# InterDigitalInc/VersatileFilmGrain

Hardware: AMD Instinct MI355X
Metric: Mpixels/s (Y+UV) + achieved HBM GB/s vs roofline, 4320p 10-bit 4:2:0 (higher is better)
Workload: dtype u16

## Files before the change

versatilefilmgrain_amd/csrc/vfgs_host.cpp:

```cpp
#include <hip/hip_runtime.h>

#include <sys/mman.h>
#include <unistd.h>

#include <algorithm>
#include <chrono>
#if defined(__SSE2__)
#include <emmintrin.h>
#endif
#include <cstdarg>
#include <cstdio>
#include <cstdlib>
#include <cstring>
#include <mutex>
#include <string>
#include <thread>
#include <vector>

#include "../../include/vfgs_hip.h"
#include "../../include/vfgs_hip_fw.h"
#include "vfgs_fw_layout.h"
#include "vfgs_layout.h"

namespace vfgs {
// ... 1211 lines not shown
	if (stride < nblk * 16 || cstride < nblk * 16 / s.csubx)
		return fail(6, "stride %u/%u too small: whole 16-sample blocks are written (need >= %u/%u)", stride, cstride, nblk * 16, nblk * 16 / s.csubx);
	if (((uintptr_t)dY | (uintptr_t)dU | (uintptr_t)dV) & 15)
		return fail(7, "plane pointers must be 16-byte aligned");
	if ((stride * sz) % 16 || (cstride * sz) % 16)
		return fail(8, "row pitch must be a multiple of 16 bytes");
	if (s.scale_shift + s.bs < 8 || s.scale_shift + s.bs > 13)
		return fail(9, "scale_shift out of range (vfgs_hw.c:170)");
	return 0;
}

void load_seed(State& s, uint32_t seed)
{
	s.lfsr.reseed(seed << 1);
	s.seed_epoch++;
	s.rnd = s.rnd_up = s.line_rnd = s.line_rnd_up = 0;
}

struct DstGeom {
	bool out8 = false;
	unsigned stride = 0, cstride = 0;
	uint64_t ypitch = 0, cpitch = 0;
};

int run_device(const void* sY, const void* sU, const void* sV, void* dY, void* dU, void* dV, unsigned width,
               unsigned frame_y, unsigned frame_h, unsigned part_y, unsigned part_h, unsigned stride, unsigned cstride,
               unsigned nframes, uint64_t ypitch, uint64_t cpitch, hipStream_t stream, DstGeom dg = DstGeom(),
               const vfgs::FrameTable* list = nullptr,
               const uint32_t* seeds = nullptr)
{
	State& s = S();
	if (list && nframes > (unsigned)vfgs::kListFrames) return fail(19, "internal: a listed launch holds at most %d frames", vfgs::kListFrames);
	if (int e = ensure_init(-1)) return e;
	if (int e = check_geometry(s, sY, sU, sV, width, stride, cstride)) return e;
	if (!dg.out8)
	{
		if (int e = check_geometry(s, dY, dU, dV, width, stride, cstride)) return e;
	}
	else
	{
		const unsigned nb = (width + 15) / 16;
		if (s.bs == 0) return fail(16, "8-bit output needs a 10- or 12-bit path (vfgs_set_depth(10) or (12))");
		if (dg.stride < nb * 16 || dg.cstride < nb * 16 / s.csubx) return fail(6, "destination stride too small");
		if ((((uintptr_t)dY | (uintptr_t)dU | (uintptr_t)dV) & 15) || dg.stride % 16 || dg.cstride % 16 || (dg.ypitch | dg.cpitch) % 16)
			return fail(8, "destination planes, pitches and frame pitches must be multiples of 16 bytes");
	}
	if (seeds && (frame_y != 0 || !list)) return fail(19, "internal: seeds belong to lists of frames that begin at line 0");
	if (part_h == 0 && seeds && nframes) load_seed(s, seeds[nframes - 1]);
	if (part_h == 0 || nframes == 0) return 0;
	if (int e = check_luts(s)) return e;

	const unsigned nblk = (width + 15) / 16;
	const unsigned sz = s.bs ? 2 : 1;
	const uint64_t crows = (uint64_t)(part_y + part_h - 1) / s.csuby - part_y / s.csuby + 1;
	const uint64_t yext = (uint64_t)part_h * stride * sz, cext = crows * cstride * sz;
	if (yext >= 0x80000000ull || cext >= 0x80000000ull)
		return fail(15, "a plane stripe of %llu bytes exceeds the 2 GiB buffer window", (unsigned long long)yext);
	KernelArgs a{};
	a.src[0] = (const uint8_t*)sY; a.src[1] = (const uint8_t*)sU; a.src[2] = (const uint8_t*)sV;
	a.dst[0] = (uint8_t*)dY; a.dst[1] = (uint8_t*)dU; a.dst[2] = (uint8_t*)dV;
	a.y0 = (int)part_y;
	a.nblk = (int)nblk;
	const int nbr_stripe = (int)(((part_y + part_h - 1) >> 4) - (part_y >> 4) + 1);
	a.nbrows = nbr_stripe;
	a.nframes = (int)nframes;
	a.listed = list ? 1 : 0;
	a.lo2[0] = (uint32_t)(s.ymin << s.bs) * 0x10001u; a.hi2[0] = (uint32_t)(s.ymax << s.bs) * 0x10001u;
	a.lo2[1] = (uint32_t)(s.cmin << s.bs) * 0x10001u; a.hi2[1] = (uint32_t)(s.cmax << s.bs) * 0x10001u;
	a.pk_shift = s.scale_shift;
	const unsigned nparts = (nblk + vfgs::kTileBlocks - 1) / vfgs::kTileBlocks;
	int rw_shrink = 0;
	bool form_one_y = false, form_one_c = false;
	digest_pluts(s);
	const bool wide = nparts > 1;
	if (image_is_current(s, wide)) { form_one_y = s.img_one_y; form_one_c = s.img_one_c; }
	else if (s.plut_bad_c < 0) image_form(s, wide, &form_one_y, &form_one_c);
	const bool mix = mix_active();
	if (mix && s.bs == 4)
		return fail(38, "a chroma mix is active and the depth is 12: the kernels of the mix exist at 8 and 10 bit");
	if (mix && !(form_one_y && form_one_c))
		return fail(38, "a chroma mix is active and the programmed model needs a general-form pattern bank (%s rows): not supported", wide ? "wide" : "ordinary");
	if (mix && &s != &g_states[0])
		return fail(38, "a chroma mix is active: not supported on the devices of vfgs_hip_init_devices");
	for (int pass = 0; pass < 3; pass++)
	{
		long waves = 0;
		for (int pt = 0; pt < 2; pt++)
		{
			vfgs::PlaneDesc& d = a.pd[pt];
			const unsigned subx = pt ? s.csubx : 1, suby = pt ? s.csuby : 1;
			const unsigned bw = 16 / subx, rpb = 16 / suby;
			d.pitch = (pt ? cstride : stride) * sz;
			d.dpitch = dg.out8 ? (pt ? dg.cstride : dg.stride) : d.pitch;
			d.fpitch = pt ? cpitch : ypitch;
			d.dfpitch = dg.out8 ? (pt ? dg.cpitch : dg.ypitch) : d.fpitch;
			d.rowbytes = nblk * bw * sz;
			d.drowbytes = dg.out8 ? nblk * bw : d.rowbytes;
			d.nrows = pt ? (int)((part_y + part_h + suby - 1) / suby) - (int)((part_y + suby - 1) / suby) : (int)part_h;
			auto lg = [](int v) { int l = 0; while ((1 << l) < v) l++; return l; };
			const int units = (int)((d.rowbytes + 15) / 16);
			d.rw_segs = (units + 1 + vfgs::kMaxUnits - 1) / vfgs::kMaxUnits;
			int rpw = 1;
			const size_t wg_bytes = (pt == 0 && s.bs == 0 && !form_one_y) ? VFGS_RW_WG_BYTES / 2 : VFGS_RW_WG_BYTES;
			while (vfgs::kWavesPerWG * rpw * 2 <= (int)rpb && (size_t)vfgs::kWavesPerWG * rpw * d.rowbytes < wg_bytes) rpw *= 2;
			for (int i = 0; i < rw_shrink && rpw > 1; i++) rpw /= 2;
			if (nparts > 1) rpw = 1;
			d.rw_rpw = rpw;
			d.rw_splits = std::max<int>(1, (int)rpb / (vfgs::kWavesPerWG * rpw));
			d.rw_lsplits = lg(d.rw_splits);
			d.wgs = d.nrows > 0 ? nbr_stripe * d.rw_splits : 0;
			waves += (long)(pt ? 2 : 1) * d.wgs * vfgs::kWavesPerWG * nframes;
		}
		const long slots = (long)s.cu_count * 16;
		if (pass < 2 && waves * 100 < VFGS_RW_MIN_FILL_PCT * slots && (a.pd[0].rw_rpw > 1 || a.pd[1].rw_rpw > 1)) { rw_shrink++; continue; }
		break;
	}

	uint64_t first_cur = 0, first_up = 0, second_cur = 0, lo = ~0ull, hi = 0;
	if (seeds)
	{
		const uint64_t b = part_y >> 4;
		first_cur = b * nblk;
		first_up = b ? (b - 1) * nblk : 0;
	}
	auto seeded_done = [&] {
		load_seed(s, seeds[nframes - 1]);
		advance_seeds(s, 0, frame_h, nblk, 0);
	};
	for (unsigned f = 0; f < nframes && f < 2 && !seeds; f++)
	{
		StripePlan p = advance_seeds(s, frame_y, frame_h, nblk, part_y);
		if (f == 0) { first_cur = p.cur0; first_up = p.up0; }
		if (f == 1) second_cur = p.cur0;
		lo = std::min(lo, std::min(p.cur0, p.up0));
		hi = std::max(hi, p.cur0 + (uint64_t)nbr_stripe * nblk);
		hi = std::max(hi, p.up0 + nblk);
	}
	if (nframes > 2 && !seeds)
	{
		if (frame_y != 0) return fail(10, "internal: a batch of stripes that do not begin at line 0");
		const uint64_t step = second_cur - first_cur, more = (uint64_t)(nframes - 2) * step;
		s.rnd += more; s.rnd_up += more; s.line_rnd += more; s.line_rnd_up += more;
		hi = std::max(hi, second_cur + more + (uint64_t)nbr_stripe * nblk);
	}
	if (int e = upload_tables(s, stream, wide)) return e;
	HIP_TRY(s.tables_ring.use(stream));
	a.tables = (const uint8_t*)s.tables_ring.current();
	const uint64_t frame_step = nframes > 1 ? second_cur - first_cur : 0;
	const uint64_t seg_bits = 32 + (uint64_t)nblk + (uint64_t)nbr_stripe * nblk + 64;
	const unsigned seg_words = (unsigned)((seg_bits + 31) / 32) + 1;
	static const bool jump_on = [] { const char* e = getenv("VFGS_HIP_STRIPE_JUMP"); return !(e && e[0] == '0'); }();
	const bool stripes = !seeds && jump_on && nframes >= 2 && first_cur >= (uint64_t)nblk + 32 && first_up + nblk + 32 >= first_cur &&
	                     (uint64_t)seg_words * 32 * 4 <= frame_step * 3;
	s.stripe_stream_last = stripes;
	s.seeded_stream_last = seeds != nullptr;
	if (seeds)
	{
		const uint64_t seg0 = first_up;
		SeededStream::Image img{};
		HIP_TRY(s.seeded.upload(seeds, nframes, seg0, seg_words, stream, &img));
		a.stream = img.dev;
		a.stream_bytes = img.words * 4;
		a.cur_bit0 = (uint32_t)(first_cur - seg0);
		a.up_bit0 = 0;
		a.frame_bit_step = seg_words * 32;
	}
	else if (stripes)
	{
		const uint64_t seg0 = first_cur - nblk - 32;
		StripeStream::Image img{};
		HIP_TRY(s.stripes.ensure(s.lfsr, seg0, frame_step, nframes, seg_words, stream, &img));
		a.stream = img.dev;
		a.stream_bytes = img.words * 4;
		a.cur_bit0 = (uint32_t)(first_cur - seg0);
		a.up_bit0 = (uint32_t)(std::max(first_up, seg0) - seg0);
		a.frame_bit_step = seg_words * 32;
	}
	else
	{
		if (int e = upload_stream(s, lo, hi, stream)) return e;
		HIP_TRY(s.lfsr.use(stream));
		a.stream = s.lfsr.dev();
		a.stream_bytes = (uint32_t)(s.lfsr.dev_words() * 4);
		a.cur_bit0 = (uint32_t)(first_cur - s.lfsr.base_bit());
		a.up_bit0 = (uint32_t)(first_up - s.lfsr.base_bit());
		a.frame_bit_step = (uint32_t)frame_step;
	}

	const long per_frame = (long)a.pd[0].wgs + 2L * a.pd[1].wgs;
	if (per_frame > 0x3fffffffL || nframes > 65535) return fail(14, "launch too large");
	if (per_frame == 0) { if (seeds) seeded_done(); return 0; }
	bool persist = false;
	long grid = per_frame;
	if (VFGS_PERSIST_MIN_TASKS > 0 && s.bs != 0 && !wide && !s.img_one_y && a.pd[0].wgs > 0 &&
	    (size_t)vfgs::kWavesPerWG * a.pd[0].rw_rpw * a.pd[0].rowbytes <= ((size_t)VFGS_PERSIST_MAX_WG_KB << 10))
	{
		const long tasks = (long)a.pd[0].wgs * nframes, slots = (long)s.cu_count * 4;
		const long k = (tasks + slots - 1) / slots;
		if (k >= VFGS_PERSIST_MIN_TASKS)
		{
			const long P = (tasks + k - 1) / k;
			persist = true;
			a.persist_wgs = (int)P;
			a.persist_step_f = (int)(P / a.pd[0].wgs);
			a.persist_step_r = (int)(P % a.pd[0].wgs);
			grid = P + 2L * a.pd[1].wgs * nframes;
			if (grid > 0x7fffffffL) return fail(14, "launch too large");
		}
	}
#ifdef VFGS_NO_FRONTS
	a.lfronts = 0;
#else
	const bool in_region = g_states[0].ov.active && (stream == g_states[0].ov.s[0] || stream == g_states[0].ov.s[1]);
	a.lfronts = (!persist && nframes >= 2 && !in_region && 2 * (yext + 2 * cext) >= (64u << 20)) ? 1 : 0;
#endif
	if (mix)
	{
		if (!(s.img_one_y && s.img_one_c) || persist) return fail(19, "internal: the table image is not the form the chroma mix was admitted for");
		a.mix_kernel = 1;
		a.mix_lw = (int)width;
		for (int c = 0; c < 2; c++)
		{
			a.mix[c][0] = g_mix[c][0]; a.mix[c][1] = g_mix[c][1];
			a.mix[c][2] = g_mix[c][2] * (1 << s.bs);
			a.mix[c][3] = g_mix[c][3];
		}
		const uint64_t dext = dg.out8 ? (uint64_t)part_h * dg.stride : yext, dfp = dg.out8 ? dg.ypitch : ypitch;
		auto meet = [](uintptr_t p, uint64_t pn, uintptr_t q, uint64_t qn) { return p < q + qn && q < p + pn; };
		bool shared = false;
		if (!list)
			shared = meet((uintptr_t)sY, (uint64_t)(nframes - 1) * ypitch + yext, (uintptr_t)dY, (uint64_t)(nframes - 1) * dfp + dext);
		else
			for (unsigned i = 0; i < nframes && !shared; i++)
				for (unsigned j = 0; j < nframes && !shared; j++)
					shared = meet((uintptr_t)list->src[0][i], yext, (uintptr_t)list->dst[0][j], dext);
		if (shared)
		{
			a.mix_planes = 1;
			HIP_TRY(vfgs::launch_grain(a, list, 8 + s.bs, s.csubx, s.csuby, dg.out8, true, true, wide, false, (int)grid, stream));
			a.mix_planes = 2;
		}
	}
	HIP_TRY(vfgs::launch_grain(a, list, 8 + s.bs, s.csubx, s.csuby, dg.out8, s.img_one_y, s.img_one_c, wide, persist, (int)grid, stream));
	if (seeds) seeded_done();
	if (stripes && s.stripes.prepare_next(s.lfsr) != hipSuccess) (void)hipGetLastError();
	if (&s == &g_states[0])
	{
		vfgs_hip_launch_info& li = g_last_launch;
		const unsigned long long n = li.launches + 1;
		li = vfgs_hip_launch_info{};
		li.launches = n;
		li.depth = 8 + s.bs; li.csubx = s.csubx; li.csuby = s.csuby;
		li.out8 = dg.out8; li.one_y = s.img_one_y; li.one_c = s.img_one_c;
		li.in_place = (sY == dY && sU == dU && sV == dV);
		li.listed = a.listed;
		li.internal = g_internal_launch ? 1 : 0;
		li.nframes = (int)nframes;
		li.workgroups_per_frame = (int)per_frame;
		li.frames_per_front = 1 << a.lfronts;
		for (int pt = 0; pt < 2; pt++)
		{
			li.rows_per_wave[pt] = a.pd[pt].rw_rpw;
			li.positions_per_row[pt] = a.pd[pt].rw_segs;
		}
		li.parts_per_row = (int)nparts;
		li.persistent_luma_workgroups = persist ? a.persist_wgs : 0;
		li.waves_per_workgroup = vfgs::kWavesPerWG;
		const vfgs::ImageLayout L = vfgs::layout_of(s.csubx, s.csuby, s.img_one_y, s.img_one_c, s.bs == 0);
		li.lds_bytes_per_workgroup = vfgs::lds_allocation(s.bs != 0, s.img_one_y, s.img_one_c, wide, L.lds_bytes + vfgs::kParamBytes);
		vfgs::describe_launch(li.kernel, sizeof li.kernel, 8 + s.bs, s.csubx, s.csuby, dg.out8, s.img_one_y, s.img_one_c, wide, persist);
		if (mix)
		{
			li.lds_bytes_per_workgroup = vfgs::mix_lds_allocation(L.lds_bytes + vfgs::kParamBytes);
			snprintf(li.kernel, sizeof li.kernel, "grain_mix_kernel<%d,%d,%d,%s,%s>", 8 + s.bs, s.csubx, s.csuby, dg.out8 ? "true" : "false", wide ? "true" : "false");
			if (a.mix_planes) li.launches++;
		}
		g_last_launch_valid = true;
	}
	return 0;
}

int run_host(void* Y, void* U, void* V, unsigned y, unsigned width, unsigned height, unsigned stride, unsigned cstride, unsigned py, unsigned ph)
{
	State& s = S();
	if (int e = ensure_init(-1)) return e;
	if (height == 0) return 0;
	const unsigned sz = s.bs ? 2 : 1;
	const unsigned nblk = (width + 15) / 16;
	if (ph == 0)
	{
		if (int e = check_luts(s)) return e;
		advance_seeds(s, y, height, nblk, y);
		return 0;
	}
	const unsigned crow0 = py / s.csuby;
	const unsigned crows = (py + ph - 1) / s.csuby - crow0 + 1;
	const unsigned rows[3] = {ph, crows, crows};
	const unsigned rowlen[3] = {nblk * 16 * sz, nblk * 16 / s.csubx * sz, nblk * 16 / s.csubx * sz};
	const unsigned dpitch[3] = {(rowlen[0] + 255) & ~255u, (rowlen[1] + 255) & ~255u, (rowlen[2] + 255) & ~255u};
	const size_t spitch[3] = {std::max<size_t>((size_t)stride * sz, rowlen[0]), std::max<size_t>((size_t)cstride * sz, rowlen[1]),
	                          std::max<size_t>((size_t)cstride * sz, rowlen[2])};
	uint8_t* host[3] = {(uint8_t*)Y + (size_t)(py - y) * spitch[0], (uint8_t*)U + (size_t)(crow0 - y / s.csuby) * spitch[1],
	                    (uint8_t*)V + (size_t)(crow0 - y / s.csuby) * spitch[2]};
	size_t total = 0;
	for (int i = 0; i < 3; i++) total += (size_t)dpitch[i] * rows[i];
	const bool via_bounce = total <= (1u << 20);
	for (int i = 0; i < 3; i++)
	{
		const size_t need = (size_t)dpitch[i] * rows[i] + 256;
		if (s.stage_cap[i] < need)
		{
			if (s.stage[i]) HIP_TRY(hipFree(s.stage[i]));
			s.stage[i] = nullptr; s.stage_cap[i] = 0;
			HIP_TRY(hipMalloc(&s.stage[i], need));
			s.stage_cap[i] = need;
		}
		if (via_bounce)
		{
			if (s.bounce_cap[i] < need)
			{
				if (s.bounce[i]) HIP_TRY(hipHostFree(s.bounce[i]));
				s.bounce[i] = nullptr; s.bounce_cap[i] = 0;
				HIP_TRY(hipHostMalloc((void**)&s.bounce[i], std::max<size_t>(need, 64u << 10), hipHostMallocDefault));
				s.bounce_cap[i] = std::max<size_t>(need, 64u << 10);
			}
			for (unsigned r = 0; r < rows[i]; r++)
				memcpy(s.bounce[i] + (size_t)r * dpitch[i], host[i] + (size_t)r * spitch[i], rowlen[i]);
			HIP_TRY(hipMemcpyAsync(s.stage[i], s.bounce[i], (size_t)dpitch[i] * rows[i], hipMemcpyHostToDevice, s.own_stream));
		}
		else
			HIP_TRY(hipMemcpy2DAsync(s.stage[i], dpitch[i], host[i], spitch[i], rowlen[i], rows[i], hipMemcpyHostToDevice, s.own_stream));
	}
	{
		InternalLaunch mark;
		if (int e = run_device(s.stage[0], s.stage[1], s.stage[2], s.stage[0], s.stage[1], s.stage[2], width, y, height, py, ph,
		                       dpitch[0] / sz, dpitch[1] / sz, 1, 0, 0, s.own_stream))
			return e;
	}
	for (int i = 0; i < 3; i++)
	{
		if (via_bounce) HIP_TRY(hipMemcpyAsync(s.bounce[i], s.stage[i], (size_t)dpitch[i] * rows[i], hipMemcpyDeviceToHost, s.own_stream));
		else HIP_TRY(hipMemcpy2DAsync(host[i], spitch[i], s.stage[i], dpitch[i], rowlen[i], rows[i], hipMemcpyDeviceToHost, s.own_stream));
	}
	HIP_TRY(hipStreamSynchronize(s.own_stream));
	if (via_bounce)
		for (int i = 0; i < 3; i++)
			for (unsigned r = 0; r < rows[i]; r++)
				memcpy(host[i] + (size_t)r * spitch[i], s.bounce[i] + (size_t)r * dpitch[i], rowlen[i]);
	return 0;
}

int run_host(void* Y, void* U, void* V, unsigned y, unsigned width, unsigned height, unsigned stride, unsigned cstride)
{
// ... 1319 lines not shown
```

versatilefilmgrain_amd/csrc/vfgs_kernel.hip:

```cpp
#include <hip/hip_runtime.h>
#include <stdint.h>
#include <stdio.h>

#include <type_traits>

#include "vfgs_layout.h"

namespace vfgs {

typedef uint32_t u32x4 __attribute__((ext_vector_type(4)));
typedef uint32_t u32x2 __attribute__((ext_vector_type(2)));
typedef uint32_t u32x3 __attribute__((ext_vector_type(3)));
typedef short s16x2 __attribute__((ext_vector_type(2)));
typedef unsigned short u16x2 __attribute__((ext_vector_type(2)));


__device__ __forceinline__ int pick_slot(uint32_t hi, uint32_t lo, uint32_t lut_entry)
{
	return (int)__builtin_amdgcn_perm(hi, lo, lut_entry) >> 24;
}

__device__ __forceinline__ int mad_i24(int x, uint32_t y, int c)
{
	int r;
// ... 870 lines not shown
#endif
template <int DEPTH, bool ONEY, bool ONEC, bool WIDE>
constexpr int rw_waves_per_simd()
{
#ifdef VFGS_ONE10_WAVES
	if (DEPTH > 8 && ONEY && ONEC && !WIDE) return VFGS_ONE10_WAVES;
#endif
	return (DEPTH == 8 && ONEY && ONEC && !WIDE && VFGS_WG_PER_CU == 4) ? (kPk16 ? VFGS_PK_WAVES : 5) : (kWavesPerWG * VFGS_WG_PER_CU + 3) / 4;
}

template <int DEPTH, int CSUBX, int CSUBY, bool OUT8, bool ONEY, bool ONEC, bool WIDE, bool PERSIST>
__global__ __launch_bounds__(kWavesPerWG * 64, (rw_waves_per_simd<DEPTH, ONEY, ONEC, WIDE>())) void grain_rw_kernel(const KernelArgs a, const FrameTable ft)
{
	constexpr ImageLayout L = image_layout(CSUBX, CSUBY, ONEY, ONEC, DEPTH == 8);
	__shared__ __attribute__((aligned(16))) uint8_t lds[lds_allocation(DEPTH > 8, ONEY, ONEC, WIDE, L.lds_bytes + kParamBytes)];

	const int lane = threadIdx.x & 63;
	const int wave = __builtin_amdgcn_readfirstlane(threadIdx.x >> 6);
	int f, r;
	if constexpr (PERSIST)
	{
		static_assert(!ONEY && !WIDE, "persistence exists for the general-form luma image");
		if ((int)blockIdx.x < a.persist_wgs)
		{
			f = (int)blockIdx.x / a.pd[0].wgs;
			r = (int)blockIdx.x - f * a.pd[0].wgs;
			run_plane_rw<DEPTH, 16, 1, 1, L.y_rs, L.y_bytes, ONEY, L.y_neg, 0, OUT8, WIDE, true>(a, ft, a.pd[0], lds, 0, f, r, L.y_off, L.y_bank, 0, lane, wave);
			return;
		}
		const int x = (int)blockIdx.x - a.persist_wgs, per = 2 * a.pd[1].wgs;
		f = x / per;
		r = a.pd[0].wgs + (x - f * per);
	}
	else
	{
		f = (int)(blockIdx.y << a.lfronts) + (int)(blockIdx.x & ((1u << a.lfronts) - 1));
		r = (int)(blockIdx.x >> a.lfronts);
	}
	if (f >= a.nframes) return;
	if (r < a.pd[0].wgs)
		run_plane_rw<DEPTH, 16, 1, 1, L.y_rs, L.y_bytes, ONEY, L.y_neg, 0, OUT8, WIDE, false>(a, ft, a.pd[0], lds, 0, f, r, L.y_off, L.y_bank, 0, lane, wave);
	else
	{
		r -= a.pd[0].wgs;
		const int comp = 1 + (r >= a.pd[1].wgs);
		if (comp == 2) r -= a.pd[1].wgs;
		if (!WIDE && CSUBX == 2 && a.pd[1].rw_segs == 2 && ring_depth<DEPTH, ONEC>() >= 2)
			run_plane_rw<DEPTH, 16 / CSUBX, CSUBX, CSUBY, L.c_rs, L.c_bytes, ONEC, L.c_neg, WIDE ? 0 : 2, OUT8, WIDE, false>(a, ft, a.pd[1], lds, comp, f, r, L.c_off[comp - 1], L.c_bank, L.c_lut[comp - 1], lane, wave);
		else if (!WIDE && CSUBX == 2 && a.pd[1].rw_segs == 1)
			run_plane_rw<DEPTH, 16 / CSUBX, CSUBX, CSUBY, L.c_rs, L.c_bytes, ONEC, L.c_neg, WIDE ? 0 : 1, OUT8, WIDE, false>(a, ft, a.pd[1], lds, comp, f, r, L.c_off[comp - 1], L.c_bank, L.c_lut[comp - 1], lane, wave);
		else
			run_plane_rw<DEPTH, 16 / CSUBX, CSUBX, CSUBY, L.c_rs, L.c_bytes, ONEC, L.c_neg, 0, OUT8, WIDE, false>(a, ft, a.pd[1], lds, comp, f, r, L.c_off[comp - 1], L.c_bank, L.c_lut[comp - 1], lane, wave);
	}
}

template <int DEPTH, int CSUBX, int CSUBY, bool OUT8, bool WIDE>
__global__ __launch_bounds__(kWavesPerWG * 64, kMixWgPerCU) void grain_mix_kernel(const KernelArgs a, const FrameTable ft)
{
	constexpr ImageLayout L = image_layout(CSUBX, CSUBY, true, true, DEPTH == 8);
	__shared__ __attribute__((aligned(16))) uint8_t lds[mix_lds_allocation(L.lds_bytes + kParamBytes)];

	const int lane = threadIdx.x & 63;
	const int wave = __builtin_amdgcn_readfirstlane(threadIdx.x >> 6);
	const int f = (int)(blockIdx.y << a.lfronts) + (int)(blockIdx.x & ((1u << a.lfronts) - 1));
	int r = (int)(blockIdx.x >> a.lfronts);
	if (f >= a.nframes) return;
	if (r < a.pd[0].wgs)
	{
		if (a.mix_planes & 1) return;
		run_plane_rw<DEPTH, 16, 1, 1, L.y_rs, L.y_bytes, true, L.y_neg, 0, OUT8, WIDE, false>(a, ft, a.pd[0], lds, 0, f, r, L.y_off, L.y_bank, 0, lane, wave);
	}
	else
	{
		if (a.mix_planes & 2) return;
		r -= a.pd[0].wgs;
		const int n = a.pd[1].wgs, full = n & ~7;
		int comp;
		if (r < 2 * full) { comp = 1 + ((r >> 3) & 1); r = ((r >> 4) << 3) | (r & 7); }
		else { r -= 2 * full; comp = 1 + (r >= n - full); r = full + (comp == 2 ? r - (n - full) : r); }
		run_plane_rw<DEPTH, 16 / CSUBX, CSUBX, CSUBY, L.c_rs, L.c_bytes, true, L.c_neg, 0, OUT8, WIDE, false, true>(a, ft, a.pd[1], lds, comp, f, r, L.c_off[comp - 1], L.c_bank, L.c_lut[comp - 1], lane, wave);
	}
}


template <int DEPTH, int CSUBX, int CSUBY, bool OUT8>
static hipError_t launch_mix(const KernelArgs& a, const FrameTable& ft, bool wide, int grid, hipStream_t stream)
{
	const dim3 g((unsigned)grid << a.lfronts, ((unsigned)a.nframes + (1u << a.lfronts) - 1) >> a.lfronts);
	if (wide)
	{
		if constexpr (CSUBX == CSUBY) hipLaunchKernelGGL((grain_mix_kernel<DEPTH, CSUBX, CSUBY, OUT8, true>), g, dim3(kWavesPerWG * 64), 0, stream, a, ft);
		else return hipErrorInvalidValue;
	}
	else
		hipLaunchKernelGGL((grain_mix_kernel<DEPTH, CSUBX, CSUBY, OUT8, false>), g, dim3(kWavesPerWG * 64), 0, stream, a, ft);
	return hipGetLastError();
}

template <int DEPTH, int CSUBX, int CSUBY, bool OUT8, bool ONEY, bool ONEC, bool WIDE, bool PERSIST>
static hipError_t launch_t(const KernelArgs& a, const FrameTable& ft, int grid, hipStream_t stream)
{
	const dim3 g = PERSIST ? dim3((unsigned)grid) : dim3((unsigned)grid << a.lfronts, ((unsigned)a.nframes + (1u << a.lfronts) - 1) >> a.lfronts);
	hipLaunchKernelGGL((grain_rw_kernel<DEPTH, CSUBX, CSUBY, OUT8, ONEY, ONEC, WIDE, PERSIST>), g, dim3(kWavesPerWG * 64), 0, stream, a, ft);
	return hipGetLastError();
}

template <int DEPTH, int CSUBX, int CSUBY, bool OUT8>
static hipError_t launch_form(const KernelArgs& a, const FrameTable& ft, bool oney, bool onec, bool wide, bool persist, int grid, hipStream_t stream)
{
	if (wide)
	{
		if (persist) return hipErrorInvalidValue;
		if constexpr (CSUBX == CSUBY)
		{
			if (oney && onec) return launch_t<DEPTH, CSUBX, CSUBY, OUT8, true, true, true, false>(a, ft, grid, stream);
			if (!oney && onec) return launch_t<DEPTH, CSUBX, CSUBY, OUT8, false, true, true, false>(a, ft, grid, stream);
		}
		return (oney || onec) ? hipErrorInvalidValue : launch_t<DEPTH, CSUBX, CSUBY, OUT8, false, false, true, false>(a, ft, grid, stream);
	}
	if constexpr (DEPTH > 8)
	{
		if (persist)
		{
			if (oney) return hipErrorInvalidValue;
			return onec ? launch_t<DEPTH, CSUBX, CSUBY, OUT8, false, true, false, true>(a, ft, grid, stream)
			            : launch_t<DEPTH, CSUBX, CSUBY, OUT8, false, false, false, true>(a, ft, grid, stream);
		}
	}
	else if (persist) return hipErrorInvalidValue;
	if (oney && onec) return launch_t<DEPTH, CSUBX, CSUBY, OUT8, true, true, false, false>(a, ft, grid, stream);
	if (oney) return launch_t<DEPTH, CSUBX, CSUBY, OUT8, true, false, false, false>(a, ft, grid, stream);
	if (onec) return launch_t<DEPTH, CSUBX, CSUBY, OUT8, false, true, false, false>(a, ft, grid, stream);
	return launch_t<DEPTH, CSUBX, CSUBY, OUT8, false, false, false, false>(a, ft, grid, stream);
}

template <int D>
static hipError_t launch_depth(const KernelArgs& a, const FrameTable& ft, int csubx, int csuby, bool out8, bool oney, bool onec, bool wide, bool persist, int grid, hipStream_t stream)
{
	if (a.mix_kernel)
	{
		if (!oney || !onec || persist) return hipErrorInvalidValue;
#define VFGS_CASE(X, Y)                                                                                  \
	if (csubx == X && csuby == Y)                                                                        \
	{                                                                                                    \
		if constexpr (D == 10) { if (out8) return launch_mix<D, X, Y, true>(a, ft, wide, grid, stream); } \
		if constexpr (D != 12) return launch_mix<D, X, Y, false>(a, ft, wide, grid, stream);              \
	}
		VFGS_CASE(2, 2) VFGS_CASE(2, 1) VFGS_CASE(1, 1) VFGS_CASE(1, 2)
#undef VFGS_CASE
		return hipErrorInvalidValue;
	}
#define VFGS_CASE(X, Y)                                                                                                     \
	if (csubx == X && csuby == Y)                                                                                           \
	{                                                                                                                       \
		if constexpr (D > 8) { if (out8) return launch_form<D, X, Y, true>(a, ft, oney, onec, wide, persist, grid, stream); }   \
		return launch_form<D, X, Y, false>(a, ft, oney, onec, wide, persist, grid, stream);                                     \
	}
	VFGS_CASE(2, 2) VFGS_CASE(2, 1) VFGS_CASE(1, 1) VFGS_CASE(1, 2)
#undef VFGS_CASE
	return hipErrorInvalidValue;
}

#if !defined(VFGS_KERNEL_DEPTH) || VFGS_KERNEL_DEPTH == 8
hipError_t launch_grain_d8(const KernelArgs& a, const FrameTable& ft, int csubx, int csuby, bool out8, bool oney, bool onec, bool wide, bool persist, int grid, hipStream_t stream)
{
	return launch_depth<8>(a, ft, csubx, csuby, out8, oney, onec, wide, persist, grid, stream);
}
#else
hipError_t launch_grain_d8(const KernelArgs& a, const FrameTable& ft, int csubx, int csuby, bool out8, bool oney, bool onec, bool wide, bool persist, int grid, hipStream_t stream);
#endif

#if !defined(VFGS_KERNEL_DEPTH) || VFGS_KERNEL_DEPTH == 12
hipError_t launch_grain_d12(const KernelArgs& a, const FrameTable& ft, int csubx, int csuby, bool out8, bool oney, bool onec, bool wide, bool persist, int grid, hipStream_t stream)
{
	return launch_depth<12>(a, ft, csubx, csuby, out8, oney, onec, wide, persist, grid, stream);
}
#else
hipError_t launch_grain_d12(const KernelArgs& a, const FrameTable& ft, int csubx, int csuby, bool out8, bool oney, bool onec, bool wide, bool persist, int grid, hipStream_t stream);
#endif

#if !defined(VFGS_KERNEL_DEPTH) || VFGS_KERNEL_DEPTH == 10
hipError_t launch_grain(const KernelArgs& a, const FrameTable* list, int depth, int csubx, int csuby, bool out8, bool oney, bool onec, bool wide, bool persist, int grid, hipStream_t stream)
{
	if ((out8 && depth != 10 && depth != 12) || wide != (a.nblk > kTileBlocks)) return hipErrorInvalidValue;
	if (a.mix_kernel ? (a.mix_lw < 1 || a.mix_lw > a.nblk * kBlock) : a.mix_planes != 0) return hipErrorInvalidValue;
	if ((a.listed != 0) != (list != nullptr) || (list && a.nframes > kListFrames)) return hipErrorInvalidValue;
	static const FrameTable no_list{};
	const FrameTable& ft = list ? *list : no_list;
	if (depth == 10) return launch_depth<10>(a, ft, csubx, csuby, out8, oney, onec, wide, persist, grid, stream);
	if (depth == 8) return launch_grain_d8(a, ft, csubx, csuby, out8, oney, onec, wide, persist, grid, stream);
	if (depth == 12) return launch_grain_d12(a, ft, csubx, csuby, out8, oney, onec, wide, persist, grid, stream);
	return hipErrorInvalidValue;
}

void describe_launch(char* out, size_t n, int depth, int csubx, int csuby, bool out8, bool oney, bool onec, bool wide, bool persist)
{
	auto b = [](bool v) { return v ? "true" : "false"; };
	snprintf(out, n, "grain_rw_kernel<%d,%d,%d,%s,%s,%s,%s,%s>", depth, csubx, csuby, b(out8), b(oney), b(onec), b(wide), b(persist));
}

ImageLayout layout_of(int csubx, int csuby, bool oney, bool onec, bool depth8) { return image_layout(csubx, csuby, oney, onec, depth8); }
#endif

}
```

versatilefilmgrain_amd/csrc/vfgs_layout.h:

```cpp
#pragma once
#include <stdint.h>

namespace vfgs {

constexpr int kSlots = 8;
constexpr int kMaxUnits = 64;
constexpr int kBlock = 16;

#ifndef VFGS_WAVES
#define VFGS_WAVES 4
#endif
#ifndef VFGS_WG_PER_CU
#define VFGS_WG_PER_CU 4
#endif
#ifndef VFGS_SCHED_FENCE
#define VFGS_SCHED_FENCE 1
#endif
#ifndef VFGS_LDAUX_ALIGNED
#define VFGS_LDAUX_ALIGNED 2
#endif
#ifndef VFGS_STAUX_ALIGNED
#define VFGS_STAUX_ALIGNED 2
#endif
#ifndef VFGS_RING
#define VFGS_RING 4
#endif
#ifndef VFGS_RING_ONE10
#define VFGS_RING_ONE10 4
#endif
#ifndef VFGS_RING_PK
#define VFGS_RING_PK 2
#endif
#ifndef VFGS_RING_NARROW10
#define VFGS_RING_NARROW10 2
#endif
#ifndef VFGS_ONE10_WG_PER_CU
#define VFGS_ONE10_WG_PER_CU 4
#endif
#ifndef VFGS_ONE8_WG_PER_CU
#define VFGS_ONE8_WG_PER_CU 0
#endif
#ifndef VFGS_RW_CONSEC
#define VFGS_RW_CONSEC 0
#endif

#if !defined(VFGS_DEV_BUILD)
#if VFGS_WAVES != 4 || VFGS_WG_PER_CU != 4 || VFGS_RING != 4 || VFGS_RING_ONE10 != 4 || VFGS_RING_PK != 2 || VFGS_RING_NARROW10 != 2 || VFGS_ONE10_WG_PER_CU != 4 || VFGS_ONE8_WG_PER_CU != 0 || VFGS_SCHED_FENCE != 1 || VFGS_LDAUX_ALIGNED != 2 || VFGS_STAUX_ALIGNED != 2 || VFGS_RW_CONSEC != 0 || \
    defined(VFGS_NO_FRONTS) || defined(VFGS_NO_LOOKAHEAD) || defined(VFGS_NO_ONE_PATTERN) || defined(VFGS_NO_PK16) || defined(VFGS_PK_NO_READ2) || defined(VFGS_PK_WAVES) || defined(VFGS_ONE10_WAVES) ||  defined(VFGS_RW_WG_BYTES) || defined(VFGS_RW_MIN_FILL_PCT) || defined(VFGS_PERSIST_MIN_TASKS) || defined(VFGS_PERSIST_MAX_WG_KB)
#error "libvfgs_hip: a tuning knob differs from the shipped configuration; developer variants must define VFGS_DEV_BUILD"
#endif
#endif

constexpr int kWavesPerWG = VFGS_WAVES;
#ifdef VFGS_NO_PK16
constexpr bool kPk16 = false;
#else
constexpr bool kPk16 = true;
#endif

constexpr int kTileBlocks = 512;
constexpr int kParamEntries = kTileBlocks + 4;
constexpr int kParamTableBytes = (kParamEntries * 4 + 15) & ~15;
constexpr int kParamBytes = 2 * kParamTableBytes;

constexpr int kLdsPerCU = 163840;
constexpr int lds_allocation(const bool depth10, const bool one_y, const bool one_c, const bool wide, const int need)
{
	const int cap = (depth10 && one_y) ? VFGS_ONE10_WG_PER_CU : ((!depth10 && one_y && one_c && !wide) ? VFGS_ONE8_WG_PER_CU : 0);
	if (cap <= 0) return need;
	const int target = (kLdsPerCU / cap) & ~2047;
	const int next = (kLdsPerCU / (cap + 1)) & ~2047;
	return need > next ? need : (target < 65536 ? target : 65536);
}

constexpr int kMixWgPerCU = 4;
constexpr int mix_lds_allocation(const int need)
{
	const int target = (kLdsPerCU / kMixWgPerCU) & ~2047;
	return need > target ? need : target;
}

struct ImageLayout {
	int lut_bytes;
	int y_rs, c_rs;
	int y_bank, c_bank;
	int y_neg, c_neg;
	int y_bytes, c_bytes;
	int y_off, c_off[2];
	int c_lut[2];
	int bytes;
	int lds_bytes;
	int cw, ch;
};

constexpr ImageLayout image_layout(int csubx, int csuby, bool one_y, bool one_c, bool depth8)
{
	ImageLayout L{};
	L.lut_bytes = 2 * 256 * 4;
	L.cw = 64 / csubx;
	L.ch = 64 / csuby;
	depth8 = depth8 && kPk16;
	const int ob = depth8 ? 2 : 1;
	L.y_rs = one_y ? 64 * ob + 16 : 64 * kSlots + 16;
	L.c_rs = one_c ? L.cw * ob + 16 : L.cw * kSlots + 16;
	L.y_bank = one_y ? (depth8 ? 256 : L.lut_bytes / 2) : L.lut_bytes;
	L.c_bank = one_c ? (depth8 ? 256 : L.lut_bytes / 2) : L.lut_bytes;
	L.y_neg = one_y ? 64 * L.y_rs : 0;
	L.c_neg = one_c ? L.ch * L.c_rs : 0;
	L.y_bytes = L.y_bank + 64 * L.y_rs + L.y_neg;
	L.c_bytes = L.c_bank + L.ch * L.c_rs + L.c_neg;
	L.y_off = 0;
	L.c_off[0] = L.y_bytes;
	L.c_off[1] = L.y_bytes + L.c_bytes;
	L.c_lut[0] = 0;
	L.c_lut[1] = 0;
	L.bytes = L.y_bytes + 2 * L.c_bytes;
	L.lds_bytes = L.y_bytes > L.c_bytes ? L.y_bytes : L.c_bytes;
	return L;
}

struct PlaneDesc {
	uint32_t pitch, dpitch;
	uint64_t fpitch, dfpitch;
	uint32_t rowbytes, drowbytes;
	int nrows;
	int wgs;
	int rw_segs;
	int rw_rpw, rw_splits, rw_lsplits;
};

constexpr int kListFrames = 32;
struct FrameTable {
	const uint8_t* src[3][kListFrames];
	uint8_t* dst[3][kListFrames];
};

struct KernelArgs {
	const uint8_t* src[3];
	uint8_t* dst[3];
	PlaneDesc pd[2];
	const uint32_t* stream;
	uint32_t stream_bytes;
	const uint8_t* tables;
	uint32_t cur_bit0;
	uint32_t up_bit0;
	uint32_t frame_bit_step;
	int y0;
	int nblk;
	int nbrows;
	int nframes;
	int listed;
	int lfronts;
	int persist_wgs;
	int persist_step_f, persist_step_r;
	int pk_shift;
	uint32_t lo2[2], hi2[2];
	int mix_kernel;
	int mix_planes;
	int mix_lw;
	int mix[2][4];
};

}
```

Measured before the change: 963,500.

## Add per-row luma workgroups for 10-bit 4:2:0 wide frames

Adds a new grain_row_kernel in which each luma workgroup handles exactly one pixel row. It loads into LDS only the bank rows that row needs (16 rows instead of the full 64-row pattern bank), which shrinks LDS per workgroup so more workgroups fit per CU (five by default). Chroma still goes through the existing row-wave path inside the same kernel. The host selects this form for 10-bit 4:2:0, general-form luma with 385 to 512 blocks per row, which covers 4320p, and disables the persistent schedule for it. In exchange, each workgroup repeats per-row setup work (bank load and block-parameter decode) 16 times per block row, and the kernel adds new DPP lane-shift code.

```diff
diff --git a/versatilefilmgrain_amd/csrc/vfgs_host.cpp b/versatilefilmgrain_amd/csrc/vfgs_host.cpp
--- a/versatilefilmgrain_amd/csrc/vfgs_host.cpp
+++ b/versatilefilmgrain_amd/csrc/vfgs_host.cpp
@@ -1317,6 +1317,7 @@
 		return fail(38, "a chroma mix is active and the programmed model needs a general-form pattern bank (%s rows): not supported", wide ? "wide" : "ordinary");
 	if (mix && &s != &g_states[0])
 		return fail(38, "a chroma mix is active: not supported on the devices of vfgs_hip_init_devices");
+	const bool rowwg = !mix && !wide && vfgs::row_form(8 + s.bs, s.csubx, s.csuby, form_one_y, dg.out8, (int)nblk);
 	for (int pass = 0; pass < 3; pass++)
 	{
 		long waves = 0;
@@ -1342,6 +1343,7 @@
 			if (nparts > 1) rpw = 1;
 			d.rw_rpw = rpw;
 			d.rw_splits = std::max<int>(1, (int)rpb / (vfgs::kWavesPerWG * rpw));
+			if (pt == 0 && rowwg) { d.rw_rpw = 1; d.rw_splits = (int)rpb; }
 			d.rw_lsplits = lg(d.rw_splits);
 			d.wgs = d.nrows > 0 ? nbr_stripe * d.rw_splits : 0;
 			waves += (long)(pt ? 2 : 1) * d.wgs * vfgs::kWavesPerWG * nframes;
@@ -1427,7 +1429,8 @@
 	if (per_frame == 0) { if (seeds) seeded_done(); return 0; }
 	bool persist = false;
 	long grid = per_frame;
-	if (VFGS_PERSIST_MIN_TASKS > 0 && s.bs != 0 && !wide && !s.img_one_y && a.pd[0].wgs > 0 &&
+	if (rowwg && s.img_one_y) return fail(19, "internal: the table image is not the form the row workgroups were chosen for");
+	if (VFGS_PERSIST_MIN_TASKS > 0 && s.bs != 0 && !wide && !rowwg && !s.img_one_y && a.pd[0].wgs > 0 &&
 	    (size_t)vfgs::kWavesPerWG * a.pd[0].rw_rpw * a.pd[0].rowbytes <= ((size_t)VFGS_PERSIST_MAX_WG_KB << 10))
 	{
 		const long tasks = (long)a.pd[0].wgs * nframes, slots = (long)s.cu_count * 4;
@@ -1476,6 +1479,7 @@
 			a.mix_planes = 2;
 		}
 	}
+	a.row_wgs = rowwg ? 1 : 0;
 	HIP_TRY(vfgs::launch_grain(a, list, 8 + s.bs, s.csubx, s.csuby, dg.out8, s.img_one_y, s.img_one_c, wide, persist, (int)grid, stream));
 	if (seeds) seeded_done();
 	if (stripes && s.stripes.prepare_next(s.lfsr) != hipSuccess) (void)hipGetLastError();
@@ -1504,6 +1508,11 @@
 		const vfgs::ImageLayout L = vfgs::layout_of(s.csubx, s.csuby, s.img_one_y, s.img_one_c, s.bs == 0);
 		li.lds_bytes_per_workgroup = vfgs::lds_allocation(s.bs != 0, s.img_one_y, s.img_one_c, wide, L.lds_bytes + vfgs::kParamBytes);
 		vfgs::describe_launch(li.kernel, sizeof li.kernel, 8 + s.bs, s.csubx, s.csuby, dg.out8, s.img_one_y, s.img_one_c, wide, persist);
+		if (rowwg)
+		{
+			li.lds_bytes_per_workgroup = vfgs::row_lds_allocation(vfgs::row_lds_need(s.img_one_c));
+			snprintf(li.kernel, sizeof li.kernel, "grain_row_kernel<%d,%s>", 8 + s.bs, s.img_one_c ? "true" : "false");
+		}
 		if (mix)
 		{
 			li.lds_bytes_per_workgroup = vfgs::mix_lds_allocation(L.lds_bytes + vfgs::kParamBytes);
diff --git a/versatilefilmgrain_amd/csrc/vfgs_kernel.hip b/versatilefilmgrain_amd/csrc/vfgs_kernel.hip
--- a/versatilefilmgrain_amd/csrc/vfgs_kernel.hip
+++ b/versatilefilmgrain_amd/csrc/vfgs_kernel.hip
@@ -976,6 +976,188 @@
 	}
 }
 
+template <int DEPTH, int RS>
+__device__ __forceinline__ void run_luma_row(const KernelArgs& a, const FrameTable& ft, uint8_t* lds, const int f, const int r,
+                                             const uint32_t img_off, const uint32_t src_bank, const uint32_t img_bytes, const int lane, const int wave)
+{
+	static_assert(DEPTH == 10, "row workgroups exist at 10 bit");
+	using M = LaneMap<8, 16>;
+	static_assert(M::PAIR && M::SHIFT * 2 / 4 == 4, "the lane shift is a whole unit");
+	constexpr int SB = kSlots;
+	constexpr int LDA = VFGS_LDAUX_ALIGNED, STA = VFGS_STAUX_ALIGNED;
+	constexpr int NU = 4;
+	constexpr int BPS = 32, SSTEP = 64;
+	constexpr uint32_t UB = kMaxUnits * 16;
+	constexpr uint32_t BANK = 2 * 256 * 4;
+	constexpr int RU = RS / 16;
+	constexpr int IMG_UNITS = (int)BANK / 16 + kRowBankRows * RU;
+	constexpr uint32_t PT_CUR = IMG_UNITS * 16, PT_UP = PT_CUR + kParamTableBytes;
+	static_assert(RS % 16 == 0, "bank rows in whole 16-byte units");
+	const PlaneDesc& pd = a.pd[0];
+	auto uni = [](int v) { return __builtin_amdgcn_readfirstlane(v); };
+
+	const int kbr = uni(r >> 4), j = uni(r & 15);
+	const int Rabs = (a.y0 >> 4) + kbr;
+	const int row = Rabs * 16 + j;
+	if (kbr >= a.nbrows || row < a.y0 || row >= a.y0 + pd.nrows) return;
+	const bool ov = Rabs > 0 && j <= 1;
+	const int last = a.nblk - 1;
+	const uint32_t cur_bit = a.cur_bit0 + (uint32_t)f * a.frame_bit_step + (uint32_t)(kbr * a.nblk);
+	const uint32_t up_bit = (kbr > 0) ? cur_bit - (uint32_t)a.nblk : a.up_bit0 + (uint32_t)f * a.frame_bit_step;
+
+	constexpr int STEP = kWavesPerWG * 64;
+	constexpr int NIT = (IMG_UNITS + STEP - 1) / STEP;
+	u32x4 tmp[NIT];
+	const __amdgpu_buffer_rsrc_t irs = make_rsrc(a.tables + img_off, img_bytes);
+#pragma unroll
+	for (int it = 0; it < NIT; it++)
+	{
+		const uint32_t i = min((uint32_t)threadIdx.x + it * STEP, (uint32_t)IMG_UNITS - 1);
+		const uint32_t bi = i - BANK / 16, c = bi / RU, col = bi - c * RU;
+		const uint32_t so = i < BANK / 16 ? i * 16 : src_bank + ((4 * c + (uint32_t)(j & 3)) * RU + col) * 16;
+		tmp[it] = __builtin_amdgcn_raw_buffer_load_b128(irs, so, 0, 0);
+	}
+	constexpr int NPE = (kParamEntries + STEP - 1) / STEP;
+	const __amdgpu_buffer_rsrc_t strs = make_rsrc((const uint8_t*)a.stream, a.stream_bytes);
+	const __amdgpu_buffer_rsrc_t strs_up = make_rsrc((const uint8_t*)a.stream, ov ? a.stream_bytes : 0);
+	u32x2 wc[NPE], wu[NPE];
+#pragma unroll
+	for (int i = 0; i < NPE; i++)
+	{
+		const int e = (int)threadIdx.x + i * STEP;
+		const uint32_t blk = (uint32_t)min(max(e - 1, 0), last);
+		const bool need = e < a.nblk + 4 && e < kParamEntries;
+		wc[i] = __builtin_amdgcn_raw_buffer_load_b64(strs, need ? ((cur_bit + blk) >> 5) * 4 : kOOB, 0, 0);
+		wu[i] = __builtin_amdgcn_raw_buffer_load_b64(strs_up, need ? ((up_bit + blk) >> 5) * 4 : kOOB, 0, 0);
+	}
+	const int tsegs = pd.rw_segs;
+	const int p0 = NU * wave;
+	const uint8_t* sbase = a.listed ? ft.src[0][f] : a.src[0] + (uint64_t)f * pd.fpitch;
+	uint8_t* dbase = a.listed ? ft.dst[0][f] : a.dst[0] + (uint64_t)f * pd.dfpitch;
+	const uint32_t ro = (uint32_t)((row - a.y0) * (int)pd.pitch);
+	const uint32_t lane16 = (uint32_t)lane * 16;
+	const uint32_t po = (uint32_t)p0 * UB;
+	const uint32_t mine = po < pd.rowbytes ? min(pd.rowbytes - po, NU * UB) : 0u;
+	const __amdgpu_buffer_rsrc_t srow = make_rsrc(sbase + ro, pd.rowbytes), drow = make_rsrc(dbase + ro, pd.rowbytes);
+	const __amdgpu_buffer_rsrc_t src = make_rsrc(sbase + ro + po, mine), dst = make_rsrc(dbase + ro + po, mine);
+	uint32_t carry[4];
+	load_seg<LDA>(srow, (lane == 0 && wave > 0) ? po - 16 : kOOB, 0, carry);
+	uint32_t w[NU][4];
+#pragma unroll
+	for (int u = 0; u < NU; u++) load_seg<LDA>(src, lane16 + u * UB, 0, w[u]);
+#pragma unroll
+	for (int it = 0; it < NIT; it++)
+		*(u32x4*)(lds + min((uint32_t)threadIdx.x + it * STEP, (uint32_t)IMG_UNITS - 1) * 16) = tmp[it];
+
+#pragma unroll
+	for (int i = 0; i < NPE; i++)
+	{
+		if (i > 0 && i * STEP >= a.nblk + 4) break;
+		const int e = (int)threadIdx.x + i * STEP;
+		const uint32_t blk = (uint32_t)min(max(e - 1, 0), last);
+		bool neg;
+		const uint32_t vc = __builtin_amdgcn_alignbit(wc[i].y, wc[i].x, (cur_bit + blk) & 31);
+		const uint32_t pc = block_param<1, 4, RS, SB>(vc, BANK, 0, 14, 31, &neg) | (neg ? 0x80000000u : 0u);
+		const uint32_t vu = __builtin_amdgcn_alignbit(wu[i].y, wu[i].x, (up_bit + blk) & 31);
+		const uint32_t pu = block_param<1, 4, RS, SB>(vu, BANK, 0, 14, 31, &neg) | (neg ? 0x80000000u : 0u);
+		if (e < kParamEntries)
+		{
+			*(uint32_t*)(lds + PT_CUR + e * 4) = pc;
+			if (ov) *(uint32_t*)(lds + PT_UP + e * 4) = pu;
+		}
+	}
+	__syncthreads();
+
+	const uint32_t lo2 = a.lo2[0], hi2 = a.hi2[0];
+	const bool first = lane & 1;
+	const uint32_t pairoff = first ? 0u : 8u * SB;
+	const uint8_t* pe = lds + ((uint32_t)(lane + 1) >> 1) * 4 + (uint32_t)(p0 * BPS * 4);
+	const int cl = lane - 1 - (lane & 1) + p0 * SSTEP;
+	const uint32_t rowoff = (uint32_t)(j >> 2) * RS, uprowoff = (uint32_t)(4 + (j >> 2)) * RS;
+	const int wc_ = j == 0 ? 12 : 24, wu_ = j == 0 ? 24 : 12;
+	auto lane_up = [](uint32_t old, uint32_t v) { return (uint32_t)__builtin_amdgcn_update_dpp((int)old, (int)v, 0x138, 0xf, 0xf, false); };
+	auto lane_down = [](uint32_t old, uint32_t v) { return (uint32_t)__builtin_amdgcn_update_dpp((int)old, (int)v, 0x130, 0xf, 0xf, false); };
+	auto rot_up = [](uint32_t v) { return (uint32_t)__builtin_amdgcn_mov_dpp((int)v, 0x13c, 0xf, 0xf, false); };
+	auto rot_down = [](uint32_t v) { return (uint32_t)__builtin_amdgcn_mov_dpp((int)v, 0x134, 0xf, 0xf, false); };
+
+	uint32_t outp[4], tp[4] = {0, 0, 0, 0};
+	auto step = [&](auto overlap, auto uc) {
+		constexpr bool OV = decltype(overlap)::value;
+		constexpr int u = decltype(uc)::value;
+		uint32_t t[4];
+		if constexpr (u < NU)
+		{
+#pragma unroll
+			for (int d = 0; d < 4; d++) t[d] = lane_up(carry[d], w[u][d]);
+#pragma unroll
+			for (int d = 0; d < 4; d++) carry[d] = rot_up(w[u][d]);
+		}
+		else
+		{
+#pragma unroll
+			for (int d = 0; d < 4; d++) t[d] = lane_up(carry[d], 0u);
+		}
+		if (p0 + u < tsegs)
+		{
+			const int jl = cl + u * SSTEP;
+			const bool edge_on[1] = {jl >= 0 && jl + 1 < 2 * a.nblk};
+			RunParam<1> rp, up;
+			const uint8_t* pu = u < NU ? pe + u * BPS * 4 : lds + min((uint32_t)(lane + 1) >> 1, (uint32_t)(kParamEntries - 1 - kTileBlocks)) * 4 + kTileBlocks * 4;
+			rp.pa[0] = *(const uint32_t*)(pu + PT_CUR) + pairoff;
+			up.pa[0] = OV ? *(const uint32_t*)(pu + PT_UP) + pairoff : 0u;
+			grain_unit<DEPTH, 16, OV, false, false, 0>(lds, t, rp, up, 0u, rowoff, uprowoff, OV ? wc_ : 0, OV ? wu_ : 0, edge_on, first, lo2, hi2, 0, t);
+		}
+#pragma unroll
+		for (int d = 0; d < 4; d++) outp[d] = lane_down(rot_down(t[d]), tp[d]);
+		if constexpr (u == 0) store_unit<4, STA>(drow, (lane == 63 && wave > 0) ? po - 16 : kOOB, outp);
+		else store_unit<4, STA>(dst, lane16 + (u - 1) * UB, outp);
+#pragma unroll
+		for (int d = 0; d < 4; d++) tp[d] = t[d];
+#if VFGS_SCHED_FENCE
+		__builtin_amdgcn_sched_barrier(0);
+#endif
+	};
+	auto walk = [&](auto overlap) {
+		step(overlap, std::integral_constant<int, 0>());
+		step(overlap, std::integral_constant<int, 1>());
+		step(overlap, std::integral_constant<int, 2>());
+		step(overlap, std::integral_constant<int, 3>());
+		if (p0 + NU < tsegs && wave == kWavesPerWG - 1)
+			step(overlap, std::integral_constant<int, 4>());
+		else
+		{
+#pragma unroll
+			for (int d = 0; d < 4; d++) outp[d] = lane_down(0u, tp[d]);
+			store_unit<4, STA>(dst, lane == 63 ? kOOB : lane16 + (NU - 1) * UB, outp);
+		}
+	};
+	if (ov) walk(std::true_type());
+	else walk(std::false_type());
+}
+
+template <int DEPTH, bool ONEC>
+__global__ __launch_bounds__(kWavesPerWG * 64, VFGS_ROW_WG_PER_CU) void grain_row_kernel(const KernelArgs a, const FrameTable ft)
+{
+	static_assert(kWavesPerWG == 4, "wave w walks positions 4w..4w+3 of a row of at most 17");
+	constexpr ImageLayout L = image_layout(2, 2, false, ONEC, false);
+	__shared__ __attribute__((aligned(16))) uint8_t lds[row_lds_allocation(row_lds_need(ONEC))];
+
+	const int lane = threadIdx.x & 63;
+	const int wave = __builtin_amdgcn_readfirstlane(threadIdx.x >> 6);
+	const int f = (int)(blockIdx.y << a.lfronts) + (int)(blockIdx.x & ((1u << a.lfronts) - 1));
+	int r = (int)(blockIdx.x >> a.lfronts);
+	if (f >= a.nframes) return;
+	if (r < a.pd[0].wgs)
+		run_luma_row<DEPTH, L.y_rs>(a, ft, lds, f, r, L.y_off, L.y_bank, L.y_bytes, lane, wave);
+	else
+	{
+		r -= a.pd[0].wgs;
+		const int comp = 1 + (r >= a.pd[1].wgs);
+		if (comp == 2) r -= a.pd[1].wgs;
+		run_plane_rw<DEPTH, 8, 2, 2, L.c_rs, L.c_bytes, ONEC, L.c_neg, 0, false, false, false>(a, ft, a.pd[1], lds, comp, f, r, L.c_off[comp - 1], L.c_bank, L.c_lut[comp - 1], lane, wave);
+	}
+}
+
 
 template <int DEPTH, int CSUBX, int CSUBY, bool OUT8>
 static hipError_t launch_mix(const KernelArgs& a, const FrameTable& ft, bool wide, int grid, hipStream_t stream)
@@ -996,6 +1178,15 @@
 {
 	const dim3 g = PERSIST ? dim3((unsigned)grid) : dim3((unsigned)grid << a.lfronts, ((unsigned)a.nframes + (1u << a.lfronts) - 1) >> a.lfronts);
 	hipLaunchKernelGGL((grain_rw_kernel<DEPTH, CSUBX, CSUBY, OUT8, ONEY, ONEC, WIDE, PERSIST>), g, dim3(kWavesPerWG * 64), 0, stream, a, ft);
+	return hipGetLastError();
+}
+
+template <int DEPTH>
+static hipError_t launch_row(const KernelArgs& a, const FrameTable& ft, bool onec, int grid, hipStream_t stream)
+{
+	const dim3 g((unsigned)grid << a.lfronts, ((unsigned)a.nframes + (1u << a.lfronts) - 1) >> a.lfronts);
+	if (onec) hipLaunchKernelGGL((grain_row_kernel<DEPTH, true>), g, dim3(kWavesPerWG * 64), 0, stream, a, ft);
+	else hipLaunchKernelGGL((grain_row_kernel<DEPTH, false>), g, dim3(kWavesPerWG * 64), 0, stream, a, ft);
 	return hipGetLastError();
 }
 
@@ -1031,6 +1222,12 @@
 template <int D>
 static hipError_t launch_depth(const KernelArgs& a, const FrameTable& ft, int csubx, int csuby, bool out8, bool oney, bool onec, bool wide, bool persist, int grid, hipStream_t stream)
 {
+	if (a.row_wgs)
+	{
+		if (a.mix_kernel || wide || persist || !row_form(D, csubx, csuby, oney, out8, a.nblk) || a.pd[0].wgs != 16 * a.nbrows) return hipErrorInvalidValue;
+		if constexpr (D == 10) return launch_row<D>(a, ft, onec, grid, stream);
+		return hipErrorInvalidValue;
+	}
 	if (a.mix_kernel)
 	{
 		if (!oney || !onec || persist) return hipErrorInvalidValue;
@@ -1076,6 +1273,7 @@
 #if !defined(VFGS_KERNEL_DEPTH) || VFGS_KERNEL_DEPTH == 10
 hipError_t launch_grain(const KernelArgs& a, const FrameTable* list, int depth, int csubx, int csuby, bool out8, bool oney, bool onec, bool wide, bool persist, int grid, hipStream_t stream)
 {
+	if (a.row_wgs && depth != 10) return hipErrorInvalidValue;
 	if ((out8 && depth != 10 && depth != 12) || wide != (a.nblk > kTileBlocks)) return hipErrorInvalidValue;
 	if (a.mix_kernel ? (a.mix_lw < 1 || a.mix_lw > a.nblk * kBlock) : a.mix_planes != 0) return hipErrorInvalidValue;
 	if ((a.listed != 0) != (list != nullptr) || (list && a.nframes > kListFrames)) return hipErrorInvalidValue;
@@ -1094,6 +1292,7 @@
 }
 
 ImageLayout layout_of(int csubx, int csuby, bool oney, bool onec, bool depth8) { return image_layout(csubx, csuby, oney, onec, depth8); }
+
 #endif
 
 }
diff --git a/versatilefilmgrain_amd/csrc/vfgs_layout.h b/versatilefilmgrain_amd/csrc/vfgs_layout.h
--- a/versatilefilmgrain_amd/csrc/vfgs_layout.h
+++ b/versatilefilmgrain_amd/csrc/vfgs_layout.h
@@ -46,7 +46,8 @@
 
 #if !defined(VFGS_DEV_BUILD)
 #if VFGS_WAVES != 4 || VFGS_WG_PER_CU != 4 || VFGS_RING != 4 || VFGS_RING_ONE10 != 4 || VFGS_RING_PK != 2 || VFGS_RING_NARROW10 != 2 || VFGS_ONE10_WG_PER_CU != 4 || VFGS_ONE8_WG_PER_CU != 0 || VFGS_SCHED_FENCE != 1 || VFGS_LDAUX_ALIGNED != 2 || VFGS_STAUX_ALIGNED != 2 || VFGS_RW_CONSEC != 0 || \
-    defined(VFGS_NO_FRONTS) || defined(VFGS_NO_LOOKAHEAD) || defined(VFGS_NO_ONE_PATTERN) || defined(VFGS_NO_PK16) || defined(VFGS_PK_NO_READ2) || defined(VFGS_PK_WAVES) || defined(VFGS_ONE10_WAVES) ||  defined(VFGS_RW_WG_BYTES) || defined(VFGS_RW_MIN_FILL_PCT) || defined(VFGS_PERSIST_MIN_TASKS) || defined(VFGS_PERSIST_MAX_WG_KB)
+    defined(VFGS_NO_FRONTS) || defined(VFGS_NO_LOOKAHEAD) || defined(VFGS_NO_ONE_PATTERN) || defined(VFGS_NO_PK16) || defined(VFGS_PK_NO_READ2) || defined(VFGS_PK_WAVES) || defined(VFGS_ONE10_WAVES) ||  defined(VFGS_RW_WG_BYTES) || defined(VFGS_RW_MIN_FILL_PCT) || defined(VFGS_PERSIST_MIN_TASKS) || defined(VFGS_PERSIST_MAX_WG_KB) || \
+    defined(VFGS_ROW_WG_PER_CU) || defined(VFGS_ROW_WORKGROUPS)
 #error "libvfgs_hip: a tuning knob differs from the shipped configuration; developer variants must define VFGS_DEV_BUILD"
 #endif
 #endif
@@ -119,6 +120,30 @@
 	return L;
 }
 
+#ifndef VFGS_ROW_WG_PER_CU
+#define VFGS_ROW_WG_PER_CU 5
+#endif
+#ifndef VFGS_ROW_WORKGROUPS
+#define VFGS_ROW_WORKGROUPS 1
+#endif
+constexpr int kRowBankRows = 16;
+constexpr int kRowMinBlocks = 385, kRowMaxBlocks = kTileBlocks;
+constexpr int row_lds_need(const bool one_c)
+{
+	const ImageLayout L = image_layout(2, 2, false, one_c, false);
+	const int luma = L.lut_bytes + kRowBankRows * L.y_rs;
+	return (luma > L.c_bytes ? luma : L.c_bytes) + kParamBytes;
+}
+constexpr int row_lds_allocation(const int need)
+{
+	const int target = (kLdsPerCU / VFGS_ROW_WG_PER_CU) & ~2047;
+	return need > target ? need : target;
+}
+constexpr bool row_form(const int depth, const int csubx, const int csuby, const bool one_y, const bool out8, const int nblk)
+{
+	return VFGS_ROW_WORKGROUPS != 0 && depth == 10 && csubx == 2 && csuby == 2 && !one_y && !out8 && nblk >= kRowMinBlocks && nblk <= kRowMaxBlocks;
+}
+
 struct PlaneDesc {
 	uint32_t pitch, dpitch;
 	uint64_t fpitch, dfpitch;
@@ -155,6 +180,7 @@
 	int persist_step_f, persist_step_r;
 	int pk_shift;
 	uint32_t lo2[2], hi2[2];
+	int row_wgs;
 	int mix_kernel;
 	int mix_planes;
 	int mix_lw;
```

After: 961,900. Within noise of the previous version (-0.2%).
